# YangYeTian/SDFace-GAN

Measured on AMD Instinct MI355X. Metric: rendered faces/sec/GPU at 256² (SDF+ngp path); 1/2/4/8-GPU scaling, higher is better.
Workload: dtype fp32

## Files before the change

### include/sdfr.h

```cpp
#ifndef SDFR_H_
#define SDFR_H_

#include <stddef.h>
#include <stdint.h>

#ifdef __cplusplus
extern "C" {
#endif

#define SDFR_OK 0
#define SDFR_EINVAL (-1)
#define SDFR_ELAUNCH (-2)
#define SDFR_EUNSUPPORTED (-3)

#define SDFR_ABI_VERSION 15

int sdfr_abi_version(void);
const char *sdfr_last_error(void);

int sdfr_grid_encode_forward(const float *inputs, const float *embeddings,
                             const int32_t *offsets, float *outputs,
                             uint32_t B, uint32_t D, uint32_t C, uint32_t L,
                             float S, uint32_t H, float *dy_dx,
                             uint32_t gridtype, int align_corners,
// ... 378 lines not shown
size_t sdfr_conv_act_ws_bytes(uint32_t B, uint32_t H, uint32_t W, uint32_t Cout);

typedef struct sdfr_conv_t_act_args {
    const void *x_split;
    const void *packed;
    uint32_t B, H, W, Cin, Cout;
    float fir[4];
    const float *demod;
    const float *noise;
    const float *noise_weight;
    const float *bias;
    float negative_slope, act_scale;
    const float *s_next;
    void *y_split;
    float *raw;
} sdfr_conv_t_act_args;
int sdfr_conv_t_act(const sdfr_conv_t_act_args *a, void *stream);
int sdfr_conv_t_act_supported(uint32_t B, uint32_t H, uint32_t W, uint32_t Cin, uint32_t Cout);

enum { SDFR_CONV_EPI_RAW = 0,
       SDFR_CONV_EPI_STYLED = 1,
       SDFR_CONV_EPI_BLUR = 2 };
enum { SDFR_CONV_K_X = 0,
       SDFR_CONV_K_X_ACT,
       SDFR_CONV_K_SPLITK,
       SDFR_CONV_K_SPLITK_ACT,
       SDFR_CONV_K_H,
       SDFR_CONV_K_H_SPLIT,
       SDFR_CONV_K_H_FINISH,
       SDFR_CONV_K_T,
       SDFR_CONV_K_T_FUSE,
       SDFR_CONV_K_T_FINISH,
       SDFR_CONV_K_T_BORDER_ROWS,
       SDFR_CONV_K_T_BORDER_COLS };
#define SDFR_CONV_PLAN_MAX_STEPS 6
typedef struct sdfr_conv_plan_query {
    uint32_t B, H, W, Cin, Cout;
    int transposed;
    int epilogue;
    int has_ws;
    size_t ws_bytes;
} sdfr_conv_plan_query;
typedef struct sdfr_conv_plan_info {
    int rc;
    uint32_t ksplit;
    uint32_t ksplit_t;
    size_t ws_bytes;
    uint32_t nsteps;
    struct { uint32_t kernel, grid_x, grid_y, block; } steps[SDFR_CONV_PLAN_MAX_STEPS];
} sdfr_conv_plan_info;
int sdfr_conv_plan(const sdfr_conv_plan_query *q, sdfr_conv_plan_info *info);

int sdfr_rgb_finish(float *rgb, const float *partial, uint32_t nparts, const float *rgb_b,
                    const float *skip, const float *fir, uint32_t B, uint32_t H, uint32_t W,
                    void *stream);

size_t sdfr_mc_workspace_bytes(uint32_t n0, uint32_t n1, uint32_t n2);
int sdfr_mc_count(const float *vol, uint32_t n0, uint32_t n1, uint32_t n2, int64_t s0,
                  int64_t s1, int64_t s2, float level, void *ws, size_t ws_bytes,
                  uint32_t *counts, void *stream);
int sdfr_mc_emit(const float *vol, uint32_t n0, uint32_t n1, uint32_t n2, int64_t s0,
                 int64_t s1, int64_t s2, float level, const void *ws, size_t ws_bytes,
                 float *verts, int32_t *faces, void *stream);

size_t sdfr_brick_layout_workspace_bytes(uint32_t nb);
int sdfr_brick_layout(const uint8_t *surface, uint32_t nb, int32_t *slots, uint32_t n_prev,
                      void *ws, size_t ws_bytes, uint32_t *n_total, void *stream);
// ... 36 lines not shown
```

### sdface-gan_amd/_lib.py

```python
from __future__ import annotations

import ctypes
import os
from pathlib import Path

PKG_DIR = Path(__file__).resolve().parent
LIB_PATH = Path(os.environ.get("SDFR_LIB", PKG_DIR / "lib" / "libsdfr.so"))

_vp = ctypes.c_void_p
_u32 = ctypes.c_uint32
_f32 = ctypes.c_float
_int = ctypes.c_int

SDFR_OK = 0
SDFR_EINVAL = -1
SDFR_ELAUNCH = -2
SDFR_EUNSUPPORTED = -3
ABI_VERSION = 15
FIELD_F16X3 = 0
FIELD_FP32 = 1

ABLATION_EXPORTS = ("sdfr_debug_set_field_variant", "sdfr_debug_set_encode_mode")
EXPORTS = (
    "sdfr_abi_version", "sdfr_last_error",
# ... 176 lines not shown
        ("dem_layer", _u32 * 16), ("dem_c", _u32 * 16), ("dem_off", _u32 * 16), ("demods", _vp),
    ]


class ConvActArgs(ctypes.Structure):
    _fields_ = [
        ("x_split", _vp), ("packed", _vp),
        ("B", _u32), ("H", _u32), ("W", _u32), ("Cin", _u32), ("Cout", _u32),
        ("demod", _vp), ("noise", _vp), ("noise_weight", _vp), ("bias", _vp),
        ("negative_slope", _f32), ("act_scale", _f32),
        ("s_next", _vp), ("y_split", _vp), ("rgb_w", _vp), ("rgb_partial", _vp),
        ("ws", _vp), ("ws_bytes", ctypes.c_size_t),
        ("rgb_base", _vp), ("rgb_s", _vp),
    ]


class ConvTActArgs(ctypes.Structure):
    _fields_ = [
        ("x_split", _vp), ("packed", _vp),
        ("B", _u32), ("H", _u32), ("W", _u32), ("Cin", _u32), ("Cout", _u32),
        ("fir", _f32 * 4),
        ("demod", _vp), ("noise", _vp), ("noise_weight", _vp), ("bias", _vp),
        ("negative_slope", _f32), ("act_scale", _f32),
        ("s_next", _vp), ("y_split", _vp), ("raw", _vp),
    ]


CONV_EPI_RAW, CONV_EPI_STYLED, CONV_EPI_BLUR = 0, 1, 2
CONV_PLAN_KERNELS = (
    "conv_x_kernel<false>", "conv_x_kernel<true>", "conv_splitk_kernel<false>",
    "conv_splitk_kernel<true>", "conv_h_kernel<false>", "conv_h_kernel<true>",
    "conv_h_finish_kernel", "conv_t_kernel<false>", "conv_t_kernel<true>",
    "conv_t_finish_kernel", "conv_t_border_kernel<true>", "conv_t_border_kernel<false>",
)


class ConvPlanQuery(ctypes.Structure):
    _fields_ = [
        ("B", _u32), ("H", _u32), ("W", _u32), ("Cin", _u32), ("Cout", _u32),
        ("transposed", _int), ("epilogue", _int), ("has_ws", _int),
        ("ws_bytes", ctypes.c_size_t),
    ]


class ConvPlanStep(ctypes.Structure):
    _fields_ = [("kernel", _u32), ("grid_x", _u32), ("grid_y", _u32), ("block", _u32)]


class ConvPlanInfo(ctypes.Structure):
    _fields_ = [
        ("rc", _int), ("ksplit", _u32), ("ksplit_t", _u32), ("ws_bytes", ctypes.c_size_t),
        ("nsteps", _u32), ("steps", ConvPlanStep * 6),
    ]


_lib = None


def lib():
    global _lib
    if _lib is not None:
        return _lib
    if not LIB_PATH.exists():
        raise RuntimeError(
            f"sdface-gan_amd: HIP library {LIB_PATH} is missing; build it with "
            "`make -C sdface-gan_amd` or `python -c 'import __graft_entry__ as g; g.build()'`")
# ... 167 lines not shown
```

### sdface-gan_amd/csrc/conv_f16x3.hip

```cpp
#include <hip/hip_runtime.h>

#include <cstdint>
#include <cstdlib>
#include <string>

#include "conv_h.h"
#include "conv_plan.h"
#include "conv_t.h"
#include "conv_x.h"
#include "sdfr_common.h"

namespace sdfr {
namespace {

__global__ void __launch_bounds__(256) conv_scale_kernel(const float *__restrict__ w, float scale,
                                                         uint32_t Cin, float *__restrict__ su) {
    const uint32_t o = blockIdx.x;
    float m = 0.0f;
    for (uint32_t k = threadIdx.x; k < Cin * 9; k += 256)
        m = fmaxf(m, fabsf(__fmul_rn(w[(size_t)o * Cin * 9 + k], scale)));
    __shared__ float red[256];
    red[threadIdx.x] = m;
    __syncthreads();
    for (uint32_t s = 128; s > 0; s >>= 1) {
// ... 13 lines not shown
    }
}

__global__ void __launch_bounds__(256) conv_pack_kernel(const float *__restrict__ w, float scale,
                                                        uint32_t Cin, uint32_t Cout,
                                                        const float *__restrict__ su,
                                                        f4 *__restrict__ packed) {
    const uint32_t e = blockIdx.x * 256 + threadIdx.x;
    const uint32_t nC = Cin / 32, nB = Cout / kCT;
    const uint32_t total = 9 * nC * nB * 8 * 64;
    if (e >= total) return;
    const uint32_t lane = e & 63, mt = (e >> 6) & 7;
    uint32_t r = e >> 9;
    const uint32_t cb = r % nB;
    r /= nB;
    const uint32_t c = r % nC, tap = r / nC;
    const uint32_t o = cb * kCT + mt * 16 + (lane & 15), g = lane >> 4;
    const float s = su[o];
    h8 H, L;
#pragma unroll
    for (int j = 0; j < 8; ++j) {
        const uint32_t i = c * 32 + 8 * g + j;
        const float v = __fmul_rn(__fmul_rn(w[((size_t)o * Cin + i) * 9 + tap], scale), s);
        H[j] = (_Float16)v;
        L[j] = (_Float16)__fsub_rn(v, (float)H[j]);
    }
    f4 *dst = packed + ((size_t)(e >> 6) * 2) * 64 + lane;
    dst[0] = __builtin_bit_cast(f4, H);
    dst[64] = __builtin_bit_cast(f4, L);
}

int conv_t_env_mode() {
    const char *e = getenv("SDFR_CONV_T");
    return e ? atoi(e) : 1;
}
int g_conv_t_mode = conv_t_env_mode();

void launch_step(const ConvStep &s, const ConvArgs &a, hipStream_t st) {
    const dim3 g(s.gx, s.gy), b(s.block);
    switch (s.kernel) {
    case kKConvX: hipLaunchKernelGGL(conv_x_kernel<false>, g, b, 0, st, a); break;
    case kKConvXAct: hipLaunchKernelGGL(conv_x_kernel<true>, g, b, 0, st, a); break;
    case kKSplitK: hipLaunchKernelGGL(conv_splitk_kernel<false>, g, b, 0, st, a); break;
    case kKSplitKAct: hipLaunchKernelGGL(conv_splitk_kernel<true>, g, b, 0, st, a); break;
    case kKConvH: hipLaunchKernelGGL(conv_h_kernel<false>, g, b, 0, st, a); break;
    case kKConvHSplit: hipLaunchKernelGGL(conv_h_kernel<true>, g, b, 0, st, a); break;
    case kKConvHFinish: hipLaunchKernelGGL(conv_h_finish_kernel, g, b, 0, st, a); break;
    case kKConvT: hipLaunchKernelGGL(conv_t_kernel<false>, g, b, 0, st, a); break;
    case kKConvTFuse: hipLaunchKernelGGL(conv_t_kernel<true>, g, b, 0, st, a); break;
    case kKConvTFinish: hipLaunchKernelGGL(conv_t_finish_kernel, g, b, 0, st, a); break;
    case kKBorderRows: hipLaunchKernelGGL(conv_t_border_kernel<true>, g, b, 0, st, a); break;
    case kKBorderCols: hipLaunchKernelGGL(conv_t_border_kernel<false>, g, b, 0, st, a); break;
    }
}

int conv_run(ConvArgs &a, const ConvShape &s, const void *x_split, const void *packed, void *ws,
             hipStream_t st, const char *what) {
    if (!x_split || !packed) return fail(SDFR_EINVAL, std::string(what) + ": null pointer");
    const ConvPlan p = plan_conv(s, g_conv_t_mode);
    if (p.rc) return fail(p.rc, std::string(what) + ": " + p.msg);
    a.xs = reinterpret_cast<const _Float16 *>(x_split);
    a.wpk = reinterpret_cast<const f4 *>(packed);
    a.B = s.B;
    a.Hin = s.H;
    a.Win = s.W;
    a.Cin = s.Cin;
    a.Cout = s.Cout;
    a.Hf = p.Hf;
    a.Wf = p.Wf;
    a.sy = p.sy;
    a.ncls = p.ncls;
    for (uint32_t i = 0; i < 4; ++i) a.cls[i] = p.cls[i];
    for (int t = 0; t < 9; ++t) {
        a.dy[t] = p.dy[t];
        a.dx[t] = p.dx[t];
        a.tap[t] = p.tap[t];
    }
    a.grid = p.grid;
    a.ksplit = p.ksplit;
    a.partial = p.ksplit > 1 ? reinterpret_cast<f4 *>(ws) : nullptr;
    a.tiles_t = p.tiles_t;
    a.ksplit_t = p.ksplit_t;
    a.ptl = p.ksplit_t > 1 ? reinterpret_cast<float *>(ws) : nullptr;
    for (uint32_t i = 0; i < p.nsteps; ++i) {
        launch_step(p.steps[i], a, st);
// ... 35 lines not shown
int sdfr_conv_pack_weights(const float *w, float scale, uint32_t Cout, uint32_t Cin,
                           void *packed, float *su, void *stream) {
    if (!w || !packed || !su) return fail(SDFR_EINVAL, "conv_pack_weights: null pointer");
    if (Cout == 0 || Cout % kCT || Cin == 0 || Cin % 32)
        return fail(SDFR_EINVAL, "conv_pack_weights: Cout % 128 and Cin % 32 must be 0");
    hipStream_t st = (hipStream_t)stream;
    hipLaunchKernelGGL(conv_scale_kernel, dim3(Cout), dim3(256), 0, st, w, scale, Cin, su);
    int rc = check_launch("conv_pack_weights: scale");
    if (rc) return rc;
    const uint32_t total = 9 * (Cin / 32) * (Cout / kCT) * 8 * 64;
    hipLaunchKernelGGL(conv_pack_kernel, dim3((total + 255) / 256), dim3(256), 0, st, w, scale,
                       Cin, Cout, su, reinterpret_cast<f4 *>(packed));
    return check_launch("conv_pack_weights: pack");
}

int sdfr_conv3x3_f16x3_ws(float *out, const void *x_split, const void *packed,
                          uint32_t B, uint32_t H, uint32_t W, uint32_t Cin, uint32_t Cout,
                          int transposed, void *ws, size_t ws_bytes, void *stream) {
    if (!out) return fail(SDFR_EINVAL, "conv3x3_f16x3: null pointer");
    ConvArgs a{};
    a.out = out;
    const ConvShape s{B, H, W, Cin, Cout, transposed != 0, kEpiRaw, ws != nullptr, ws_bytes};
    return conv_run(a, s, x_split, packed, ws, (hipStream_t)stream, "conv3x3_f16x3");
}

int sdfr_conv3x3_f16x3(float *out, const void *x_split, const void *packed,
                       uint32_t B, uint32_t H, uint32_t W, uint32_t Cin, uint32_t Cout,
                       int transposed, void *stream) {
    return sdfr_conv3x3_f16x3_ws(out, x_split, packed, B, H, W, Cin, Cout, transposed, nullptr, 0,
                                 stream);
}

int sdfr_set_conv_t_mode(int mode) {
    if (mode < -1 || mode > 3) return fail(SDFR_EINVAL, "set_conv_t_mode: mode must be -1..3");
    const int prev = g_conv_t_mode;
    g_conv_t_mode = mode == -1 ? conv_t_env_mode() : mode;
    return prev;
}

size_t sdfr_conv_ws_bytes(uint32_t B, uint32_t H, uint32_t W, uint32_t Cout, int transposed) {
    return plan_ws_bytes(B, H, W, Cout, transposed != 0, kEpiRaw);
}

size_t sdfr_conv_act_ws_bytes(uint32_t B, uint32_t H, uint32_t W, uint32_t Cout) {
    return plan_ws_bytes(B, H, W, Cout, false, kEpiStyled);
}

int sdfr_conv_plan(const sdfr_conv_plan_query *q, sdfr_conv_plan_info *info) {
    if (!q || !info) return fail(SDFR_EINVAL, "conv_plan: null argument");
    const ConvShape s{q->B, q->H, q->W, q->Cin, q->Cout, q->transposed != 0, q->epilogue,
                      q->has_ws != 0, q->ws_bytes};
    const ConvPlan p = plan_conv(s, g_conv_t_mode);
    *info = sdfr_conv_plan_info{};
    info->rc = p.rc;
    info->ksplit = p.ksplit;
    info->ksplit_t = p.ksplit_t;
    info->ws_bytes = p.ws_bytes;
    info->nsteps = p.nsteps;
    for (uint32_t i = 0; i < p.nsteps; ++i) {
        info->steps[i].kernel = p.steps[i].kernel;
        info->steps[i].grid_x = p.steps[i].gx;
        info->steps[i].grid_y = p.steps[i].gy;
        info->steps[i].block = p.steps[i].block;
    }
    return p.rc ? fail(p.rc, std::string("conv_plan: ") + p.msg) : SDFR_OK;
}

// ... 6 lines not shown
    if (s.rgb_w && s.rgb_base) return fail(SDFR_EINVAL, "conv3x3_f16x3_act: rgb_w and rgb_base are exclusive");
    if (s.rgb_base && !s.rgb_s) return fail(SDFR_EINVAL, "conv3x3_f16x3_act: rgb_base needs rgb_s");
    if (!s.y_split && !rgb) return fail(SDFR_EINVAL, "conv3x3_f16x3_act: nothing to write");
    if (rgb && !s.rgb_partial) return fail(SDFR_EINVAL, "conv3x3_f16x3_act: rgb_partial missing");
    if (((uint64_t)s.H * s.W) % kPT)
        return fail(SDFR_EUNSUPPORTED, "conv3x3_f16x3_act: H*W must be a multiple of 256");
    for (const void *q : {(const void *)s.demod, (const void *)s.bias, (const void *)s.s_next,
                          (const void *)s.rgb_w, (const void *)s.y_split, (const void *)s.rgb_base,
                          (const void *)s.rgb_s})
        if (q && reinterpret_cast<uintptr_t>(q) % 16)
            return fail(SDFR_EINVAL, "conv3x3_f16x3_act: pointers must be 16-B aligned");
    ConvArgs a{};
    set_act_epilogue(a.e, s.demod, s.noise, s.noise_weight, s.bias, s.negative_slope, s.act_scale,
                     s.s_next, s.y_split);
    a.e.rgb_w = s.rgb_w;
    a.e.rgbp = s.rgb_partial;
    a.e.rgb_base = s.rgb_base;
    a.e.rgb_s = s.rgb_s;
    const ConvShape sh{s.B, s.H, s.W, s.Cin, s.Cout, false, kEpiStyled, s.ws != nullptr, s.ws_bytes};
    return conv_run(a, sh, s.x_split, s.packed, s.ws, (hipStream_t)stream, "conv3x3_f16x3_act");
}

int sdfr_conv_t_act_supported(uint32_t B, uint32_t H, uint32_t W, uint32_t Cin, uint32_t Cout) {
    const ConvShape s{B, H, W, Cin, Cout, true, kEpiBlur, false, 0};
    return plan_conv(s, g_conv_t_mode).rc != SDFR_EUNSUPPORTED;
}

int sdfr_conv_t_act(const sdfr_conv_t_act_args *p, void *stream) {
    if (!p) return fail(SDFR_EINVAL, "conv_t_act: null args");
    const sdfr_conv_t_act_args &s = *p;
    if (!s.demod || !s.bias || !s.y_split || !s.raw || (s.noise && !s.noise_weight))
        return fail(SDFR_EINVAL, "conv_t_act: null tensor pointer");
    for (const void *q : {(const void *)s.demod, (const void *)s.bias, (const void *)s.s_next,
                          (const void *)s.y_split, (const void *)s.raw, (const void *)s.noise})
        if (q && reinterpret_cast<uintptr_t>(q) % 16)
            return fail(SDFR_EINVAL, "conv_t_act: pointers must be 16-B aligned");
    ConvArgs a{};
    a.out = s.raw;
    set_act_epilogue(a.e, s.demod, s.noise, s.noise_weight, s.bias, s.negative_slope, s.act_scale,
                     s.s_next, s.y_split);
    for (int k = 0; k < 4; ++k) a.fir[k] = s.fir[k];
    const ConvShape sh{s.B, s.H, s.W, s.Cin, s.Cout, true, kEpiBlur, false, 0};
    return conv_run(a, sh, s.x_split, s.packed, nullptr, (hipStream_t)stream, "conv_t_act");
}

}
```

### sdface-gan_amd/csrc/conv_plan.h

```cpp
#pragma once

#include <cstddef>
#include <cstdint>

#include "../../include/sdfr.h"

namespace sdfr {

constexpr int kCT = 128;
constexpr int kPT = 256;
constexpr uint32_t kTCT = 64;
constexpr uint32_t kCusPerXcd = 32;
constexpr size_t kPartialTileBytes = 16 * 512 * 16;

struct ConvClass {
    uint32_t Hc, Wc;
    uint32_t py, px;
    uint32_t a0, c0;
    uint32_t ntaps, t0;
    uint32_t tile0, ntiles;
    uint32_t td[3];
};

enum ConvEpilogue : int {
    kEpiRaw = SDFR_CONV_EPI_RAW,
    kEpiStyled = SDFR_CONV_EPI_STYLED,
    kEpiBlur = SDFR_CONV_EPI_BLUR,
};

struct ConvShape {
    uint32_t B, H, W, Cin, Cout;
    bool transposed;
    int epi;
    bool has_ws;
    size_t ws_bytes;
};

enum ConvKernel : uint32_t {
    kKConvX = SDFR_CONV_K_X,
    kKConvXAct = SDFR_CONV_K_X_ACT,
    kKSplitK = SDFR_CONV_K_SPLITK,
    kKSplitKAct = SDFR_CONV_K_SPLITK_ACT,
    kKConvH = SDFR_CONV_K_H,
    kKConvHSplit = SDFR_CONV_K_H_SPLIT,
    kKConvHFinish = SDFR_CONV_K_H_FINISH,
    kKConvT = SDFR_CONV_K_T,
    kKConvTFuse = SDFR_CONV_K_T_FUSE,
    kKConvTFinish = SDFR_CONV_K_T_FINISH,
    kKBorderRows = SDFR_CONV_K_T_BORDER_ROWS,
    kKBorderCols = SDFR_CONV_K_T_BORDER_COLS,
};

struct ConvStep {
    uint32_t kernel;
    uint32_t gx, gy, block;
};
constexpr uint32_t kMaxConvSteps = SDFR_CONV_PLAN_MAX_STEPS;

struct ConvPlan {
    int rc;
    const char *msg;
    uint32_t Hf, Wf, sy;
    uint32_t ncls, ntap;
    ConvClass cls[4];
    int dy[9], dx[9];
    uint32_t tap[9];
    uint32_t grid;
    uint32_t ksplit;
    uint32_t tiles_t;
    uint32_t ksplit_t;
    size_t ws_bytes;
    uint32_t nsteps;
    ConvStep steps[kMaxConvSteps];
};

constexpr uint32_t kKsplitMax = 320;
inline uint32_t conv_ksplit(uint32_t grid) {
    for (uint32_t k = 4; k > 1; --k)
        if (grid * k <= kKsplitMax) return k;
    return 1;
}

inline uint32_t conv_h_grid(uint32_t ntiles) {
    const uint32_t per = (ntiles + 7) >> 3;
    return 8u * (per < kCusPerXcd ? per : kCusPerXcd);
}

inline ConvPlan plan_refuse(ConvPlan p, int rc, const char *msg) {
    p.rc = rc;
    p.msg = msg;
    p.nsteps = 0;
    return p;
}

inline void plan_step(ConvPlan &p, ConvKernel k, uint32_t gx, uint32_t gy, uint32_t block) {
    p.steps[p.nsteps++] = ConvStep{k, gx, gy, block};
}

inline void plan_tap(ConvPlan &p, int ky, int kx, bool transposed) {
    p.dy[p.ntap] = transposed ? -(ky >> 1) : ky - 1;
    p.dx[p.ntap] = transposed ? -(kx >> 1) : kx - 1;
    p.tap[p.ntap] = (uint32_t)(ky * 3 + kx);
    ++p.ntap;
}

inline void plan_class(ConvPlan &p, const ConvShape &s, uint32_t Hc, uint32_t Wc, uint32_t py,
                       uint32_t px, uint32_t nt, uint32_t a0 = 0, uint32_t c0 = 0) {
    ConvClass &c = p.cls[p.ncls++];
    c.Hc = Hc;
    c.Wc = Wc;
    c.py = py;
    c.px = px;
    c.a0 = a0;
    c.c0 = c0;
    c.t0 = p.ntap - nt;
    c.ntaps = nt;
    c.tile0 = p.grid;
    c.ntiles = (s.B * Hc * Wc + kPT - 1) / kPT * (s.Cout / kCT);
    p.grid += (c.ntiles + 7) & ~7u;
    for (uint32_t t = 0; t < nt; ++t) {
        const uint32_t d = p.tap[c.t0 + t] | (uint32_t)(p.dy[c.t0 + t] + 1) << 4 |
                           (uint32_t)(p.dx[c.t0 + t] + 1) << 6;
        c.td[t >> 2] |= d << (8 * (t & 3u));
    }
}

inline void plan_conv_t(ConvPlan &p, const ConvShape &s) {
    const uint32_t B = s.B, H = s.H, W = s.W, Cout = s.Cout;
    const bool fuse = s.epi == kEpiBlur;
    plan_tap(p, 2, 0, true), plan_tap(p, 2, 2, true);
    plan_class(p, s, 1, W + 1, 0, 0, 2, H, 0);
    plan_tap(p, 2, 1, true);
    plan_class(p, s, 1, W, 0, 1, 1, H, 0);
    plan_tap(p, 0, 2, true), plan_tap(p, 2, 2, true);
    plan_class(p, s, H, 1, 0, 0, 2, 0, W);
    plan_tap(p, 1, 2, true);
    plan_class(p, s, H, 1, 1, 0, 1, 0, W);
    plan_step(p, fuse ? kKConvTFuse : kKConvT, conv_h_grid(p.tiles_t * p.ksplit_t), 1, 512);
    if (p.ksplit_t > 1) {
        const uint64_t n4 = (uint64_t)B * 4 * H * W * (Cout / 4);
        plan_step(p, kKConvTFinish, (uint32_t)((n4 + 255) / 256), 1, 256);
    }
    plan_step(p, kKConvX, p.grid, 1, 512);
    if (fuse) {
        const uint32_t H2 = 2u * H, W2 = 2u * W;
        const uint64_t nr = (uint64_t)B * (H2 / 32u + 1u) * (W2 / 4u) * (Cout / 4u);
        const uint64_t nc = (uint64_t)B * (H2 / 4u) * (W2 / 32u + 1u) * (Cout / 4u);
        plan_step(p, kKBorderRows, (uint32_t)((nr + 255) / 256), 1, 256);
        plan_step(p, kKBorderCols, (uint32_t)((nc + 255) / 256), 1, 256);
    }
}

inline void plan_strips(ConvPlan &p, const ConvShape &s) {
    const bool act = s.epi == kEpiStyled;
    const uint32_t ks = conv_ksplit(p.grid);
    p.ws_bytes = ks > 1 ? (size_t)ks * p.grid * kPartialTileBytes : 0;
    if (s.has_ws && ks > 1 && s.ws_bytes >= p.ws_bytes) p.ksplit = ks;
    if (act && s.H % 16 == 0 && s.W % 16 == 0) {
        while (p.ksplit > 1 && (s.Cin / 32) % p.ksplit) --p.ksplit;
        const uint32_t nt = p.cls[0].ntiles;
        if (p.ksplit > 1) {
            plan_step(p, kKConvHSplit, conv_h_grid(nt * p.ksplit), 1, 512);
            plan_step(p, kKConvHFinish, nt, 4, 128);
        } else {
            plan_step(p, kKConvH, conv_h_grid(nt), 1, 512);
        }
        return;
    }
    plan_step(p, act ? kKConvXAct : kKConvX, p.grid, p.ksplit, 512);
    if (p.ksplit > 1) plan_step(p, act ? kKSplitKAct : kKSplitK, p.grid, 1, 512);
}

inline ConvPlan plan_conv(const ConvShape &s, int mode) {
    ConvPlan p{};
    p.ksplit = p.ksplit_t = 1;
    const uint32_t B = s.B, H = s.H, W = s.W, Cin = s.Cin, Cout = s.Cout;
    const bool blur = s.epi == kEpiBlur;
    const char *below = "shape below conv_t_kernel's range (sdfr_conv_t_act_supported)";
    if (s.epi < kEpiRaw || s.epi > kEpiBlur || (blur && !s.transposed) ||
        (s.epi == kEpiStyled && s.transposed))
        return plan_refuse(p, SDFR_EINVAL, "the epilogue does not go with this conv form");
    if (B == 0 || H == 0 || W == 0 || Cout % kCT || Cin % 32 || Cin == 0 || Cout == 0)
        return blur ? plan_refuse(p, SDFR_EUNSUPPORTED, below)
                    : plan_refuse(p, SDFR_EINVAL, "bad shape (Cout % 128, Cin % 32)");
    const uint64_t tiles = (uint64_t)B * (H / 16) * (W / 16) * (Cout / kTCT);
    const bool conv_t = s.transposed && mode != 0 && H % 16 == 0 && W % 16 == 0 &&
                        (tiles >= 256 || mode >= 2);
    if (blur && !conv_t) return plan_refuse(p, SDFR_EUNSUPPORTED, below);
    p.Hf = s.transposed ? 2 * H + 1 : H;
    p.Wf = s.transposed ? 2 * W + 1 : W;
    p.sy = s.transposed ? 2 : 1;
    if ((uint64_t)B * H * W * Cin * 4 >= (1ull << 31) || 9ull * Cin * Cout * 4 >= (1ull << 31) ||
        (uint64_t)B * H * W * Cout * 4 >= (1ull << 31) ||
        (blur && (uint64_t)B * p.Hf * p.Wf * Cout * 4 >= (1ull << 31)))
        return plan_refuse(p, SDFR_EINVAL, "tensor too large for 32-bit offsets (split B)");
    if (conv_t) {
        p.tiles_t = (uint32_t)tiles;
        if (mode == 3 && !blur && tiles < 256) {
            for (uint32_t k = 4; k > 1 && p.ws_bytes == 0; k /= 2)
                if (tiles * k <= 256) p.ws_bytes = (size_t)k * B * p.Hf * p.Wf * Cout * sizeof(float);
            for (uint32_t k = 4; k > 1 && p.ksplit_t == 1; k /= 2)
                if (s.has_ws && s.ws_bytes >= p.ws_bytes && tiles * k <= 256 && Cin / 32 >= 2 * k)
                    p.ksplit_t = k;
        }
        plan_conv_t(p, s);
    } else if (s.transposed) {
        for (uint32_t py = 0; py < 2; ++py)
            for (uint32_t px = 0; px < 2; ++px) {
                uint32_t nt = 0;
                for (int ky = (int)py; ky < 3; ky += 2)
                    for (int kx = (int)px; kx < 3; kx += 2, ++nt) plan_tap(p, ky, kx, true);
                plan_class(p, s, py ? H : H + 1, px ? W : W + 1, py, px, nt);
            }
        plan_strips(p, s);
    } else {
        for (int t = 0; t < 9; ++t) plan_tap(p, t / 3, t % 3, false);
        plan_class(p, s, H, W, 0, 0, 9);
        plan_strips(p, s);
    }
    return p;
}

}
```

### sdface-gan_amd/csrc/conv_t.h

```cpp
#pragma once

#include "conv_common.h"

namespace sdfr {
namespace {

__host__ __device__ constexpr int t_ky(int s) {
    return (s == 2 || s == 3 || s == 7) ? 1 : ((s == 4 || s == 5 || s == 8) ? 2 : 0);
}
__host__ __device__ constexpr int t_kx(int s) { return s < 6 ? (s & 1) : 2; }
__host__ __device__ constexpr int t_pos(int s) { return s < 4 ? 0 : (s < 6 ? 1 : (s < 8 ? 2 : 3)); }

__device__ __forceinline__ bool t_band(uint32_t r) { return r <= 2u || r >= 29u; }
__device__ __forceinline__ bool t_border(uint32_t r) { return r == 0u || r >= 30u; }

template <bool PREV>
__device__ __forceinline__ f4 dpp_row_shift(f4 v) {
    typedef int i4 __attribute__((ext_vector_type(4)));
    constexpr int ctl = PREV ? 0x111 : 0x101;
    const i4 iv = __builtin_bit_cast(i4, v);
    i4 r;
    r.x = __builtin_amdgcn_update_dpp(0, iv.x, ctl, 0xF, 0xF, true);
    r.y = __builtin_amdgcn_update_dpp(0, iv.y, ctl, 0xF, 0xF, true);
    r.z = __builtin_amdgcn_update_dpp(0, iv.z, ctl, 0xF, 0xF, true);
    r.w = __builtin_amdgcn_update_dpp(0, iv.w, ctl, 0xF, 0xF, true);
    return __builtin_bit_cast(f4, r);
}

__device__ __forceinline__ void store_split8_pair_if(_Float16 *ys, size_t idx8, f4 v, uint32_t g,
                                                     bool live) {
    asm volatile("" : "+v"(v));
    h4 h, l;
#pragma unroll
    for (int r = 0; r < 4; ++r) {
        h[r] = (_Float16)v[r];
// ... 111 lines not shown
                    store_split8_pair_if(e.ys, P * C + (ch & ~7u), v * sn, g,
                                         !t_border(yr) && !t_border(xr));
                }
                __builtin_amdgcn_sched_barrier(0);
            }
    }
}

__device__ __forceinline__ f4 border_ld(const float *src, int yy, int xx, uint32_t Hi, uint32_t Wi,
                                        uint32_t C) {
    return (yy >= 0 && yy < (int)Hi && xx >= 0 && xx < (int)Wi)
               ? *reinterpret_cast<const f4 *>(src + ((size_t)yy * Wi + xx) * C)
               : f4{0.0f, 0.0f, 0.0f, 0.0f};
}

__device__ __forceinline__ void border_out(const ConvArgs &a, uint32_t b, uint32_t Y, uint32_t X,
                                           uint32_t c, f4 s, const f4 &dm, const f4 &bs,
                                           const f4 &sn, float nw) {
    const ActEpi &e = a.e;
    const uint32_t C = a.Cout, H2 = 2u * a.Hin, W2 = 2u * a.Win;
    const size_t P = ((size_t)b * H2 + Y) * W2 + X;
    const float nz = e.noise ? nw * e.noise[P] : 0.0f;
    f4 v;
#pragma unroll
    for (int r = 0; r < 4; ++r) v[r] = act1(s[r], dm[r], nz, bs[r], e.slope, e.scale);
    v = v * sn;
    asm volatile("" : "+v"(v));
    h4 hh, ll;
#pragma unroll
    for (int r = 0; r < 4; ++r) {
        hh[r] = (_Float16)v[r];
        ll[r] = (_Float16)(v[r] - (float)hh[r]);
    }
    const size_t idx = P * C + c, o = 2 * idx - (idx & 7u);
    *reinterpret_cast<h4 *>(e.ys + o) = hh;
    *reinterpret_cast<h4 *>(e.ys + o + 8) = ll;
}

template <bool ROWS>
__global__ void __launch_bounds__(256) conv_t_border_kernel(const ConvArgs a) {
    const uint32_t Q = a.Cout >> 2, H2 = 2u * a.Hin, W2 = 2u * a.Win;
    const uint32_t kb = H2 / 32u + 1u, mb = W2 / 32u + 1u;
    const uint32_t items = ROWS ? kb * (W2 / 4u) : (H2 / 4u) * mb;
    const uint64_t t = (uint64_t)blockIdx.x * 256u + threadIdx.x;
    if (t >= (uint64_t)a.B * items * Q) return;
    const uint32_t q = (uint32_t)(t % Q);
    const uint64_t r1 = t / Q;
    const uint32_t item = (uint32_t)(r1 % items);
    const uint32_t b = (uint32_t)(r1 / items);
    const uint32_t c = 4u * q, C = a.Cout, Hi = a.Hf, Wi = a.Wf;
    const float *src = a.out + (size_t)b * Hi * Wi * C + c;
    const float f0 = a.fir[3], f1 = a.fir[2], f2 = a.fir[1], f3 = a.fir[0];
    const ActEpi &e = a.e;
    const f4 dm = *reinterpret_cast<const f4 *>(e.demod + (size_t)b * C + c);
    const f4 bs = *reinterpret_cast<const f4 *>(e.bias + c);
    const f4 sn = e.s_next ? *reinterpret_cast<const f4 *>(e.s_next + (size_t)b * C + c)
                           : f4{1.0f, 1.0f, 1.0f, 1.0f};
    const float nw = e.noise ? *e.noise_weight : 0.0f;
    if constexpr (ROWS) {
        const uint32_t k = item / (W2 / 4u), X0 = 4u * (item % (W2 / 4u));
        const int Yb = 32 * (int)k - 2;
        f4 h[4][4];
#pragma unroll
        for (int r = 0; r < 6; ++r) {
            f4 v[7];
#pragma unroll
            for (int j = 0; j < 7; ++j) v[j] = border_ld(src, Yb - 1 + r, (int)X0 - 1 + j, Hi, Wi, C);
#pragma unroll
            for (int x = 0; x < 4; ++x)
                h[r & 3][x] = fir_h(v[x], v[x + 1], v[x + 2], v[x + 3], f0, f1, f2, f3);
            if (r >= 3) {
                const int y = r - 3, Y = Yb + y;
                if (Y >= 0 && Y < (int)H2) {
#pragma unroll
                    for (int x = 0; x < 4; ++x)
                        border_out(a, b, (uint32_t)Y, X0 + x, c,
                                   fir_v(h[y & 3][x], h[(y + 1) & 3][x], h[(y + 2) & 3][x],
                                         h[(y + 3) & 3][x], f0, f1, f2, f3),
                                   dm, bs, sn, nw);
                }
            }
            __builtin_amdgcn_sched_barrier(0);
        }
    } else {
        const uint32_t m = item % mb, Y0 = 4u * (item / mb);
        const int Xb = 32 * (int)m - 2;
        f4 h[4][3];
#pragma unroll
        for (int r = 0; r < 7; ++r) {
            f4 v[6];
#pragma unroll
            for (int j = 0; j < 6; ++j) v[j] = border_ld(src, (int)Y0 - 1 + r, Xb - 1 + j, Hi, Wi, C);
#pragma unroll
            for (int x = 0; x < 3; ++x)
                h[r & 3][x] = fir_h(v[x], v[x + 1], v[x + 2], v[x + 3], f0, f1, f2, f3);
            if (r >= 3) {
                const int y = r - 3;
                const uint32_t Y = Y0 + y, yb = Y & 31u;
                if (yb != 0u && yb < 30u) {
#pragma unroll
                    for (int x = 0; x < 3; ++x) {
                        const int X = Xb + x;
                        if (X < 0 || X >= (int)W2) continue;
                        border_out(a, b, Y, (uint32_t)X, c,
                                   fir_v(h[y & 3][x], h[(y + 1) & 3][x], h[(y + 2) & 3][x],
                                         h[(y + 3) & 3][x], f0, f1, f2, f3),
                                   dm, bs, sn, nw);
                    }
                }
            }
            __builtin_amdgcn_sched_barrier(0);
        }
    }
}

template <bool FUSE>
__global__ void __launch_bounds__(512, 1) conv_t_kernel(const ConvArgs a) {
    __shared__ f4 As[3][kTStepF4];
    __shared__ f4 Hs[2][kHaloF4];
    __shared__ f4 Ep[FUSE ? 7 * 64 : 1];
    const uint32_t tid = threadIdx.x, lane = tid & 63u;
    const uint32_t wave = __builtin_amdgcn_readfirstlane(tid >> 6);
    const uint32_t wm = wave & 1u, wn = wave >> 1;
    const uint32_t H = a.Hin, W = a.Win;
    const uint32_t nC = a.Cin / 32, nB = a.Cout / kCT, nT = a.Cout / kTCT;
    const uint32_t nbx = W / 16, nby = H / 16;
    const v4i rw = make_rsrc(a.wpk, 9u * nC * nB * kStepF4 * 16u);
    const v4i rx = make_rsrc(a.xs, a.B * H * W * a.Cin * 4);
    const uint32_t ks = a.ksplit_t;
    uint32_t cb = 0, bimg = 0, y0 = 0, x0 = 0, split = 0, cg0 = 0, cg1 = 0, hoff[6];
    auto setup = [&](uint32_t item) {
        uint32_t ln = lane, wv = wave;
        asm volatile("" : "+v"(ln), "+s"(wv));
        const uint32_t tile = item / ks;
        split = item - tile * ks;
        cg0 = split * nC / ks;
        cg1 = (split + 1) * nC / ks;
        cb = tile % nT;
        uint32_t blk = tile / nT;
        const uint32_t bx = blk % nbx;
        blk /= nbx;
        const uint32_t by = blk % nby, b = blk / nby;
        bimg = b;
        y0 = by * 16;
        x0 = bx * 16;
// ... 237 lines not shown
```

### sdface-gan_amd/decoder_ops.py

```python
from __future__ import annotations

import math

import torch
import torch.nn as nn
import torch.nn.functional as F
from torch.autograd import Function

from . import _lib


def _require_cuda(*ts):
    for t in ts:
        if t is not None and not t.is_cuda:
            raise RuntimeError(f"{tuple(t.shape)} must be a CUDA tensor")


def fused_bias_act(input, bias, refer, act, grad, alpha, scale):
    _require_cuda(input, bias)
    x = input.contiguous()
    b = bias.contiguous() if bias is not None and bias.numel() else None
    r = refer.contiguous() if refer is not None and refer.numel() else None
    out = torch.empty_like(x)
    step_b = 1
# ... 306 lines not shown
        if t is None:
            return None
        t = t.contiguous()
        keep.append(t)
        return _lib.ptr(t)

    a = _lib.ConvActArgs()
    a.x_split, a.packed = _lib.ptr(x_split), _lib.ptr(packed)
    a.B, a.H, a.W, a.Cin, a.Cout = B, H, W, Cin, Cout
    a.demod = cptr(demod)
    a.noise = cptr(noise)
    a.noise_weight = cptr(noise_weight)
    a.bias = cptr(bias.reshape(-1))
    a.negative_slope, a.act_scale = negative_slope, act_scale
    a.s_next = cptr(s_next)
    a.y_split = _lib.ptr(ys)
    a.rgb_w = cptr(rgb_w)
    a.rgb_base = cptr(rgb_base)
    a.rgb_s = cptr(rgb_s)
    a.rgb_partial = _lib.ptr(part)
    wsb = _lib.lib().sdfr_conv_act_ws_bytes(B, H, W, Cout) if split_k else 0
    ws = torch.empty(wsb, dtype=torch.uint8, device=dev) if wsb else None
    a.ws, a.ws_bytes = _lib.ptr(ws), wsb
    _lib.check(_lib.lib().sdfr_conv3x3_f16x3_act(a, _lib.stream_of(x_split)), "conv3x3_f16x3_act")
    return ys, part


def conv_t_act_supported(x_split, Cout):
    B, H, W, Cin = x_split.shape[0], x_split.shape[1], x_split.shape[2], 8 * x_split.shape[3]
    return bool(_lib.lib().sdfr_conv_t_act_supported(B, H, W, Cin, Cout))


def conv_t_act(x_split, packed, Cout, *, fir, demod, bias, noise_weight, noise=None,
               s_next=None, negative_slope=0.2, act_scale=math.sqrt(2)):
    _require_cuda(x_split)
    if x_split.dtype != torch.float16 or x_split.dim() != 6 or x_split.shape[4:] != (2, 8) \
            or not x_split.is_contiguous():
        raise RuntimeError("conv_t_act: x_split must be a contiguous split-NHWC fp16 "
                           "tensor [B,H,W,Cin/8,2,8]")
    B, H, W, Cin = x_split.shape[0], x_split.shape[1], x_split.shape[2], 8 * x_split.shape[3]
    dev = x_split.device
    ys = torch.empty(B, 2 * H, 2 * W, Cout // 8, 2, 8, device=dev, dtype=torch.float16)
    raw = torch.empty(B, 2 * H + 1, 2 * W + 1, Cout, device=dev)
    if noise is not None:
        noise = noise.expand(B, 1, 2 * H, 2 * W).contiguous()
    keep = []

    def cptr(t):
        if t is None:
            return None
        t = t.contiguous()
        keep.append(t)
        return _lib.ptr(t)

    a = _lib.ConvTActArgs()
    a.x_split, a.packed = _lib.ptr(x_split), _lib.ptr(packed)
    a.B, a.H, a.W, a.Cin, a.Cout = B, H, W, Cin, Cout
    for i in range(4):
        a.fir[i] = fir[i]
    a.demod = cptr(demod)
    a.noise = cptr(noise)
    a.noise_weight = cptr(noise_weight)
    a.bias = cptr(bias.reshape(-1))
    a.negative_slope, a.act_scale = negative_slope, act_scale
    a.s_next = cptr(s_next)
    a.y_split = _lib.ptr(ys)
    a.raw = _lib.ptr(raw)
    _lib.check(_lib.lib().sdfr_conv_t_act(a, _lib.stream_of(x_split)), "conv_t_act")
    return ys


def rgb_finish(partial, rgb_b, skip=None, fir=None):
    _require_cuda(partial)
    n, B, _, H, W = partial.shape
    partial = partial.contiguous()
    rgb = torch.empty(B, 3, H, W, device=partial.device)
# ... 20 lines not shown
```

Baseline: 3326.

## Add edge-tile conv kernel and merged seam pass for fused transposed conv

Adds a default seam mode (mode 4) for the fused blur transposed conv. In this mode the edge pixel classes run in a dedicated small-tile (32-pixel) MFMA kernel instead of the general conv_x kernel, and the two border blur passes (rows and columns) are merged into one XCD-swizzled launch. The split-fp16 store in the epilogue now exchanges halves across lanes with DPP, so each lane writes one 16-byte vector instead of two 8-byte ones. The column border indexing is reordered and the caller can pass in a preallocated raw buffer. This is meant to cut launch count and wasted tile work on the thin edge classes, at the risk of lower MFMA utilisation in the new edge kernel and correctness concerns in the new index mapping.

```diff
diff --git a/include/sdfr.h b/include/sdfr.h
--- a/include/sdfr.h
+++ b/include/sdfr.h
@@ -434,7 +434,9 @@
        SDFR_CONV_K_T_FUSE,
        SDFR_CONV_K_T_FINISH,
        SDFR_CONV_K_T_BORDER_ROWS,
-       SDFR_CONV_K_T_BORDER_COLS };
+       SDFR_CONV_K_T_BORDER_COLS,
+       SDFR_CONV_K_T_EDGE,
+       SDFR_CONV_K_T_SEAM };
 #define SDFR_CONV_PLAN_MAX_STEPS 6
 typedef struct sdfr_conv_plan_query {
     uint32_t B, H, W, Cin, Cout;
diff --git a/sdface-gan_amd/_lib.py b/sdface-gan_amd/_lib.py
--- a/sdface-gan_amd/_lib.py
+++ b/sdface-gan_amd/_lib.py
@@ -232,6 +232,7 @@
     "conv_splitk_kernel<true>", "conv_h_kernel<false>", "conv_h_kernel<true>",
     "conv_h_finish_kernel", "conv_t_kernel<false>", "conv_t_kernel<true>",
     "conv_t_finish_kernel", "conv_t_border_kernel<true>", "conv_t_border_kernel<false>",
+    "conv_t_edge_kernel", "conv_t_seam_kernel",
 )
 
 
diff --git a/sdface-gan_amd/csrc/conv_f16x3.hip b/sdface-gan_amd/csrc/conv_f16x3.hip
--- a/sdface-gan_amd/csrc/conv_f16x3.hip
+++ b/sdface-gan_amd/csrc/conv_f16x3.hip
@@ -69,7 +69,7 @@
 
 int conv_t_env_mode() {
     const char *e = getenv("SDFR_CONV_T");
-    return e ? atoi(e) : 1;
+    return e ? atoi(e) : 4;
 }
 int g_conv_t_mode = conv_t_env_mode();
 
@@ -88,6 +88,8 @@
     case kKConvTFinish: hipLaunchKernelGGL(conv_t_finish_kernel, g, b, 0, st, a); break;
     case kKBorderRows: hipLaunchKernelGGL(conv_t_border_kernel<true>, g, b, 0, st, a); break;
     case kKBorderCols: hipLaunchKernelGGL(conv_t_border_kernel<false>, g, b, 0, st, a); break;
+    case kKConvTEdge: hipLaunchKernelGGL(conv_t_edge_kernel, g, b, 0, st, a); break;
+    case kKConvTSeam: hipLaunchKernelGGL(conv_t_seam_kernel, g, b, 0, st, a); break;
     }
 }
 
@@ -189,7 +191,7 @@
 }
 
 int sdfr_set_conv_t_mode(int mode) {
-    if (mode < -1 || mode > 3) return fail(SDFR_EINVAL, "set_conv_t_mode: mode must be -1..3");
+    if (mode < -1 || mode > 5) return fail(SDFR_EINVAL, "set_conv_t_mode: mode must be -1..5");
     const int prev = g_conv_t_mode;
     g_conv_t_mode = mode == -1 ? conv_t_env_mode() : mode;
     return prev;
@@ -262,7 +264,8 @@
     if (!s.demod || !s.bias || !s.y_split || !s.raw || (s.noise && !s.noise_weight))
         return fail(SDFR_EINVAL, "conv_t_act: null tensor pointer");
     for (const void *q : {(const void *)s.demod, (const void *)s.bias, (const void *)s.s_next,
-                          (const void *)s.y_split, (const void *)s.raw, (const void *)s.noise})
+                          (const void *)s.y_split, (const void *)s.raw, (const void *)s.noise,
+                          s.x_split, s.packed})
         if (q && reinterpret_cast<uintptr_t>(q) % 16)
             return fail(SDFR_EINVAL, "conv_t_act: pointers must be 16-B aligned");
     ConvArgs a{};
diff --git a/sdface-gan_amd/csrc/conv_plan.h b/sdface-gan_amd/csrc/conv_plan.h
--- a/sdface-gan_amd/csrc/conv_plan.h
+++ b/sdface-gan_amd/csrc/conv_plan.h
@@ -10,6 +10,7 @@
 constexpr int kCT = 128;
 constexpr int kPT = 256;
 constexpr uint32_t kTCT = 64;
+constexpr uint32_t kEdgePT = 32;
 constexpr uint32_t kCusPerXcd = 32;
 constexpr size_t kPartialTileBytes = 16 * 512 * 16;
 
@@ -49,6 +50,8 @@
     kKConvTFinish = SDFR_CONV_K_T_FINISH,
     kKBorderRows = SDFR_CONV_K_T_BORDER_ROWS,
     kKBorderCols = SDFR_CONV_K_T_BORDER_COLS,
+    kKConvTEdge = SDFR_CONV_K_T_EDGE,
+    kKConvTSeam = SDFR_CONV_K_T_SEAM,
 };
 
 struct ConvStep {
@@ -105,7 +108,8 @@
 }
 
 inline void plan_class(ConvPlan &p, const ConvShape &s, uint32_t Hc, uint32_t Wc, uint32_t py,
-                       uint32_t px, uint32_t nt, uint32_t a0 = 0, uint32_t c0 = 0) {
+                       uint32_t px, uint32_t nt, uint32_t a0 = 0, uint32_t c0 = 0,
+                       uint32_t pt = kPT) {
     ConvClass &c = p.cls[p.ncls++];
     c.Hc = Hc;
     c.Wc = Wc;
@@ -116,7 +120,7 @@
     c.t0 = p.ntap - nt;
     c.ntaps = nt;
     c.tile0 = p.grid;
-    c.ntiles = (s.B * Hc * Wc + kPT - 1) / kPT * (s.Cout / kCT);
+    c.ntiles = (s.B * Hc * Wc + pt - 1) / pt * (s.Cout / kCT);
     p.grid += (c.ntiles + 7) & ~7u;
     for (uint32_t t = 0; t < nt; ++t) {
         const uint32_t d = p.tap[c.t0 + t] | (uint32_t)(p.dy[c.t0 + t] + 1) << 4 |
@@ -125,29 +129,35 @@
     }
 }
 
-inline void plan_conv_t(ConvPlan &p, const ConvShape &s) {
+inline void plan_conv_t(ConvPlan &p, const ConvShape &s, bool seam) {
     const uint32_t B = s.B, H = s.H, W = s.W, Cout = s.Cout;
     const bool fuse = s.epi == kEpiBlur;
+    const uint32_t pt = fuse && seam ? kEdgePT : (uint32_t)kPT;
     plan_tap(p, 2, 0, true), plan_tap(p, 2, 2, true);
-    plan_class(p, s, 1, W + 1, 0, 0, 2, H, 0);
+    plan_class(p, s, 1, W + 1, 0, 0, 2, H, 0, pt);
     plan_tap(p, 2, 1, true);
-    plan_class(p, s, 1, W, 0, 1, 1, H, 0);
+    plan_class(p, s, 1, W, 0, 1, 1, H, 0, pt);
     plan_tap(p, 0, 2, true), plan_tap(p, 2, 2, true);
-    plan_class(p, s, H, 1, 0, 0, 2, 0, W);
+    plan_class(p, s, H, 1, 0, 0, 2, 0, W, pt);
     plan_tap(p, 1, 2, true);
-    plan_class(p, s, H, 1, 1, 0, 1, 0, W);
+    plan_class(p, s, H, 1, 1, 0, 1, 0, W, pt);
     plan_step(p, fuse ? kKConvTFuse : kKConvT, conv_h_grid(p.tiles_t * p.ksplit_t), 1, 512);
     if (p.ksplit_t > 1) {
         const uint64_t n4 = (uint64_t)B * 4 * H * W * (Cout / 4);
         plan_step(p, kKConvTFinish, (uint32_t)((n4 + 255) / 256), 1, 256);
     }
-    plan_step(p, kKConvX, p.grid, 1, 512);
-    if (fuse) {
-        const uint32_t H2 = 2u * H, W2 = 2u * W;
-        const uint64_t nr = (uint64_t)B * (H2 / 32u + 1u) * (W2 / 4u) * (Cout / 4u);
-        const uint64_t nc = (uint64_t)B * (H2 / 4u) * (W2 / 32u + 1u) * (Cout / 4u);
-        plan_step(p, kKBorderRows, (uint32_t)((nr + 255) / 256), 1, 256);
-        plan_step(p, kKBorderCols, (uint32_t)((nc + 255) / 256), 1, 256);
+    if (fuse && seam) plan_step(p, kKConvTEdge, p.grid, 1, 256);
+    else plan_step(p, kKConvX, p.grid, 1, 512);
+    if (!fuse) return;
+    const uint32_t H2 = 2u * H, W2 = 2u * W;
+    const uint64_t nr = (uint64_t)B * (H2 / 32u + 1u) * (W2 / 4u) * (Cout / 4u);
+    const uint64_t nc = (uint64_t)B * (H2 / 4u) * (W2 / 32u + 1u) * (Cout / 4u);
+    const uint32_t rblocks = (uint32_t)((nr + 255) / 256), cblocks = (uint32_t)((nc + 255) / 256);
+    if (seam) {
+        plan_step(p, kKConvTSeam, (rblocks + cblocks + 7) & ~7u, 1, 256);
+    } else {
+        plan_step(p, kKBorderRows, rblocks, 1, 256);
+        plan_step(p, kKBorderCols, cblocks, 1, 256);
     }
 }
 
@@ -171,7 +181,9 @@
     if (p.ksplit > 1) plan_step(p, act ? kKSplitKAct : kKSplitK, p.grid, 1, 512);
 }
 
-inline ConvPlan plan_conv(const ConvShape &s, int mode) {
+inline ConvPlan plan_conv(const ConvShape &s, int mode_seam) {
+    const bool seam = mode_seam >= 4;
+    const int mode = seam ? mode_seam - 3 : mode_seam;
     ConvPlan p{};
     p.ksplit = p.ksplit_t = 1;
     const uint32_t B = s.B, H = s.H, W = s.W, Cin = s.Cin, Cout = s.Cout;
@@ -203,7 +215,7 @@
                 if (s.has_ws && s.ws_bytes >= p.ws_bytes && tiles * k <= 256 && Cin / 32 >= 2 * k)
                     p.ksplit_t = k;
         }
-        plan_conv_t(p, s);
+        plan_conv_t(p, s, seam);
     } else if (s.transposed) {
         for (uint32_t py = 0; py < 2; ++py)
             for (uint32_t px = 0; px < 2; ++px) {
diff --git a/sdface-gan_amd/csrc/conv_t.h b/sdface-gan_amd/csrc/conv_t.h
--- a/sdface-gan_amd/csrc/conv_t.h
+++ b/sdface-gan_amd/csrc/conv_t.h
@@ -1,6 +1,7 @@
 #pragma once
 
 #include "conv_common.h"
+#include "conv_x.h"
 
 namespace sdfr {
 namespace {
@@ -178,17 +179,24 @@
         hh[r] = (_Float16)v[r];
         ll[r] = (_Float16)(v[r] - (float)hh[r]);
     }
-    const size_t idx = P * C + c, o = 2 * idx - (idx & 7u);
-    *reinterpret_cast<h4 *>(e.ys + o) = hh;
-    *reinterpret_cast<h4 *>(e.ys + o + 8) = ll;
+    typedef uint32_t u2 __attribute__((ext_vector_type(2)));
+    typedef uint32_t u4 __attribute__((ext_vector_type(4)));
+    const u2 hd = __builtin_bit_cast(u2, hh), ld = __builtin_bit_cast(u2, ll);
+    const bool odd = (c & 4u) != 0u;
+    const u2 give = odd ? hd : ld;
+    u2 got;
+    got.x = (uint32_t)__builtin_amdgcn_update_dpp(0, (int)give.x, 0xB1, 0xF, 0xF, true);
+    got.y = (uint32_t)__builtin_amdgcn_update_dpp(0, (int)give.y, 0xB1, 0xF, 0xF, true);
+    const u4 st = odd ? u4{got.x, got.y, ld.x, ld.y} : u4{hd.x, hd.y, got.x, got.y};
+    const size_t idx8 = P * C + (c & ~7u);
+    *reinterpret_cast<u4 *>(e.ys + 2 * idx8 + (odd ? 8u : 0u)) = st;
 }
 
 template <bool ROWS>
-__global__ void __launch_bounds__(256) conv_t_border_kernel(const ConvArgs a) {
+__device__ __forceinline__ void seam_thread(const ConvArgs &a, uint64_t t) {
     const uint32_t Q = a.Cout >> 2, H2 = 2u * a.Hin, W2 = 2u * a.Win;
     const uint32_t kb = H2 / 32u + 1u, mb = W2 / 32u + 1u;
     const uint32_t items = ROWS ? kb * (W2 / 4u) : (H2 / 4u) * mb;
-    const uint64_t t = (uint64_t)blockIdx.x * 256u + threadIdx.x;
     if (t >= (uint64_t)a.B * items * Q) return;
     const uint32_t q = (uint32_t)(t % Q);
     const uint64_t r1 = t / Q;
@@ -229,7 +237,7 @@
             __builtin_amdgcn_sched_barrier(0);
         }
     } else {
-        const uint32_t m = item % mb, Y0 = 4u * (item / mb);
+        const uint32_t m = item / (H2 / 4u), Y0 = 4u * (item % (H2 / 4u));
         const int Xb = 32 * (int)m - 2;
         f4 h[4][3];
 #pragma unroll
@@ -257,6 +265,112 @@
             }
             __builtin_amdgcn_sched_barrier(0);
         }
+    }
+}
+
+template <bool ROWS>
+__global__ void __launch_bounds__(256) conv_t_border_kernel(const ConvArgs a) {
+    seam_thread<ROWS>(a, (uint64_t)blockIdx.x * 256u + threadIdx.x);
+}
+
+__global__ void __launch_bounds__(256) conv_t_seam_kernel(const ConvArgs a) {
+    const uint32_t Q = a.Cout >> 2, H2 = 2u * a.Hin, W2 = 2u * a.Win;
+    const uint64_t nr = (uint64_t)a.B * (H2 / 32u + 1u) * (W2 / 4u) * Q;
+    const uint32_t rblocks = (uint32_t)((nr + 255u) / 256u);
+    const uint32_t bid = (blockIdx.x & 7u) * (gridDim.x >> 3) + (blockIdx.x >> 3);
+    if (bid < rblocks) seam_thread<true>(a, (uint64_t)bid * 256u + threadIdx.x);
+    else seam_thread<false>(a, (uint64_t)(bid - rblocks) * 256u + threadIdx.x);
+}
+
+constexpr uint32_t kEdgeUnroll = 4;
+__global__ void __launch_bounds__(256) conv_t_edge_kernel(const ConvArgs a) {
+    const uint32_t lane = threadIdx.x & 63u;
+    const uint32_t wave = __builtin_amdgcn_readfirstlane(threadIdx.x >> 6);
+    uint32_t ci, tile;
+    if (!slot_tile(a, blockIdx.x, ci, tile)) return;
+    const ConvClass &cl = a.cls[ci];
+    const uint32_t Hc = cl.Hc, Wc = cl.Wc, ntaps = cl.ntaps;
+    const uint32_t npix = a.B * Hc * Wc;
+    const uint32_t nC = a.Cin / 32, nB = a.Cout / kCT;
+    const uint32_t cb = tile % nB, pix0 = (tile / nB) * kEdgePT;
+    const uint32_t n = lane & 15u, g = lane >> 4;
+    const uint32_t td0 = cl.td[0];
+    uint32_t xoff[2], tmask[2];
+#pragma unroll
+    for (int j = 0; j < 2; ++j) {
+        const uint32_t P = pix0 + 16u * j + n;
+        const bool pv = P < npix;
+        const uint32_t Pc = pv ? P : 0, hw = Hc * Wc;
+        const uint32_t pb = Pc / hw, rem = Pc % hw, pa = rem / Wc + cl.a0, pc = rem % Wc + cl.c0;
+        xoff[j] = ((pb * a.Hin + pa) * a.Win + pc) * a.Cin * 4u + g * 32u;
+        uint32_t m = 0;
+        for (uint32_t t = 0; t < ntaps; ++t) {
+            const uint32_t d = (td0 >> (8 * t)) & 0xFFu;
+            const int iy = (int)pa + (int)((d >> 4) & 3u) - 1, ix = (int)pc + (int)(d >> 6) - 1;
+            if (pv && iy >= 0 && iy < (int)a.Hin && ix >= 0 && ix < (int)a.Win) m |= 1u << t;
+        }
+        tmask[j] = m;
+    }
+    const char *xs = reinterpret_cast<const char *>(a.xs);
+    const f4 zero = {0.0f, 0.0f, 0.0f, 0.0f};
+    f4 acc[2][2];
+#pragma unroll
+    for (int i = 0; i < 2; ++i)
+#pragma unroll
+        for (int j = 0; j < 2; ++j) acc[i][j] = zero;
+    const uint32_t nk = nC * ntaps;
+    uint32_t c = 0, t = 0;
+    for (uint32_t k0 = 0; k0 < nk; k0 += kEdgeUnroll) {
+        f4 A[kEdgeUnroll][4], Bf[kEdgeUnroll][4];
+#pragma unroll
+        for (uint32_t u = 0; u < kEdgeUnroll; ++u) {
+            if (k0 + u < nk) {
+                const uint32_t d = (td0 >> (8 * t)) & 0xFFu;
+                const f4 *w = a.wpk + (size_t)(((d & 15u) * nC + c) * nB + cb) * kStepF4 +
+                              4u * wave * 64u + lane;
+                A[u][0] = w[0];
+                A[u][2] = w[64];
+                A[u][1] = w[128];
+                A[u][3] = w[192];
+                const int dy = (int)((d >> 4) & 3u) - 1, dx = (int)(d >> 6) - 1;
+                const uint32_t toff = (uint32_t)((dy * (int)a.Win + dx) * (int)a.Cin * 4) + c * 128u;
+#pragma unroll
+                for (int j = 0; j < 2; ++j) {
+                    const bool ok = (tmask[j] >> t) & 1u;
+                    const f4 *x = reinterpret_cast<const f4 *>(xs + (ok ? xoff[j] + toff : g * 32u));
+                    const f4 hi = x[0], lo = x[1];
+                    Bf[u][j] = ok ? hi : zero;
+                    Bf[u][2 + j] = ok ? lo : zero;
+                }
+                const bool wrap = t + 1 == ntaps;
+                t = wrap ? 0u : t + 1;
+                c = wrap ? c + 1 : c;
+            }
+        }
+#pragma unroll
+        for (uint32_t u = 0; u < kEdgeUnroll; ++u) {
+            if (k0 + u < nk) {
+#pragma unroll
+                for (int i = 0; i < 2; ++i) {
+#pragma unroll
+                    for (int j = 0; j < 2; ++j) acc[i][j] = mfma16(A[u][2 + i], Bf[u][j], acc[i][j]);
+#pragma unroll
+                    for (int j = 0; j < 2; ++j) acc[i][j] = mfma16(A[u][i], Bf[u][2 + j], acc[i][j]);
+#pragma unroll
+                    for (int j = 0; j < 2; ++j) acc[i][j] = mfma16(A[u][i], Bf[u][j], acc[i][j]);
+                }
+            }
+        }
+    }
+#pragma unroll
+    for (int j = 0; j < 2; ++j) {
+        const uint32_t P = pix0 + 16u * j + n;
+        if (P >= npix) continue;
+        const uint32_t hw = Hc * Wc, b = P / hw, rem = P % hw;
+        const uint32_t oy = a.sy * (rem / Wc + cl.a0) + cl.py, ox = a.sy * (rem % Wc + cl.c0) + cl.px;
+        float *dst = a.out + (((size_t)b * a.Hf + oy) * a.Wf + ox) * a.Cout + cb * kCT + 4 * g;
+#pragma unroll
+        for (int i = 0; i < 2; ++i) *reinterpret_cast<f4 *>(dst + (2 * wave + i) * 16) = acc[i][j];
     }
 }
 
diff --git a/sdface-gan_amd/decoder_ops.py b/sdface-gan_amd/decoder_ops.py
--- a/sdface-gan_amd/decoder_ops.py
+++ b/sdface-gan_amd/decoder_ops.py
@@ -362,7 +362,7 @@
 
 
 def conv_t_act(x_split, packed, Cout, *, fir, demod, bias, noise_weight, noise=None,
-               s_next=None, negative_slope=0.2, act_scale=math.sqrt(2)):
+               s_next=None, negative_slope=0.2, act_scale=math.sqrt(2), raw=None):
     _require_cuda(x_split)
     if x_split.dtype != torch.float16 or x_split.dim() != 6 or x_split.shape[4:] != (2, 8) \
             or not x_split.is_contiguous():
@@ -371,7 +371,11 @@
     B, H, W, Cin = x_split.shape[0], x_split.shape[1], x_split.shape[2], 8 * x_split.shape[3]
     dev = x_split.device
     ys = torch.empty(B, 2 * H, 2 * W, Cout // 8, 2, 8, device=dev, dtype=torch.float16)
-    raw = torch.empty(B, 2 * H + 1, 2 * W + 1, Cout, device=dev)
+    if raw is None:
+        raw = torch.empty(B, 2 * H + 1, 2 * W + 1, Cout, device=dev)
+    elif raw.shape != (B, 2 * H + 1, 2 * W + 1, Cout) or raw.dtype != torch.float32 \
+            or not raw.is_contiguous() or raw.device != dev:
+        raise RuntimeError("conv_t_act: raw must be a contiguous fp32 [B,2H+1,2W+1,Cout] tensor")
     if noise is not None:
         noise = noise.expand(B, 1, 2 * H, 2 * W).contiguous()
     keep = []
```

New measurement: 3318 (median of 2 runs). No clear change (-0.3%).
